# zrudnick/bramble

Hardware: AMD Instinct MI355X
Metric: projected alignments/sec vs GENCODE-scale annotation (higher is better)
Workload: dtype u32; 1 GPU; device-resident (inputs already in HBM, packed rows left in HBM): 10M paired-end 2x100 short reads (name-collated, unstranded) vs GENCODE-shaped synthetic annotation (250836 transcripts, 1684128 transcript-exon rows, 25 refs); BASELINE.json configs[1]; group_lanes=8, seed=0xb4a3b1e

## Files before the change

### bramble_amd/csrc/kernels.h

```cpp
#pragma once
#include <hip/hip_runtime.h>
#include <stdint.h>

#include "device_types.h"
#include "ksw_types.h"

namespace br {

enum {
  TOT_MATCHES = 0,
  TOT_ARENA = 1,
  TOT_SIMPLE = 2,
  TOT_ROWS = 3,
  TOT_RAW = 4,
  TOT_RESCUE_PROB = 5,
  TOT_RESCUE_SEQ = 6,
  TOT_WIDE_CIGAR = 7,
  TOT_SMALL_CNT = 8,
  TOT_PARSE_CIGAR = 12,
  TOT_PARSE_NAMES = 13,
  TOT_PARSE_GROUPS = 14,
  TOT_PARSE_SEQ = 15,
  TOT_BAM_LONG = 16,
  TOT_BAM_BYTES = 17,
// ... 6 lines not shown

struct ProjectArgs {
  DevIndex ix;
  DevCfg cfg;
  int64_t n_aln;
  const int32_t *ref_id;
  const uint32_t *cigar_off;
  const uint32_t *cigar;
  const uint2 *seg;
  const AlnMeta *meta;
  const uint4 *head;
  const uint4 *head2;
  const uint32_t *fast_flag;
  const uint32_t *fast_pre;
  uint32_t *n_matches;
  uint4 *ranges;
  uint64_t *mask;
  uint32_t *big_list;
  uint32_t *n_big;
  uint32_t *walk_list;
  uint32_t *n_walk;
  uint32_t *m_aln;
  const uint32_t *match_off;
  const uint64_t *cig_base;
  uint32_t *m_tid, *m_aux;
  uint2 *m_p;
  uint2 *m_x;
  uint4 *m_b;
  uint64_t *m_cigoff;
  uint32_t *cig_arena;
  const uint64_t *tot;
  uint64_t lim_m, lim_c;
  uint64_t cover;
};
__device__ __forceinline__ bool tot_over(const uint64_t *tot, uint64_t lim_m, uint64_t lim_c) { return tot && (tot[TOT_MATCHES] > lim_m || tot[TOT_ARENA] > lim_c); }

struct CountArgs {
  const uint32_t *slab_off, *bin_off, *s_start, *s_pmax;
  const uint4 *t_bin, *s_row, *tx_ex;
  uint32_t n_refs, bin_shift;
  uint32_t max_clip, max_junc_ins, max_junc_gap, max_error_exon;
  int32_t ignore_small_exons, long_reads;
  uint32_t n_aln;
  const uint4 *head, *head2;
  const uint32_t *cigar_off;
  const uint2 *seg;
  uint32_t *n_matches;
  uint64_t *mask;
  uint4 *ranges;
  uint32_t *walk_list, *n_walk;
  uint32_t *big_list, *n_big;
  uint32_t *light_flag;
};

struct FaArgs {
  const int32_t *seq_src;
  const uint32_t *seq_off;
  const uint8_t *seqs;
  uint32_t *n_prob;
  uint32_t *seq_bytes;
  const uint32_t *prob_off;
  const uint64_t *seqarena_off;
  KswProb *probs;
  FaSrc *srcs;
  KswRes *results;
  uint8_t *seq_arena;
  uint32_t *clip_ops;
  uint32_t *ideal_cap;
  uint64_t *want_l, *want_r;
};

struct KswArgs {
  int64_t n_prob;
  const KswProb *probs;
  KswRes *results;
  const uint8_t *seq_arena;
  uint32_t *clip_ops;
  uint8_t *scratch;
  size_t scratch_per_wave, pmat_bytes, raw_words;
  int64_t n_waves;
  uint32_t tmax;
  uint64_t *stats;
  uint32_t *raw_out, *raw_n; int32_t *max_out; uint32_t raw_cap;
  const uint32_t *list; const uint32_t *n_list;
};

struct KswFastArgs {
  int64_t p0, n;
  const KswProb *probs;
  KswRes *results;
  const uint8_t *seq_arena;
  uint32_t *clip_ops, *raw_ops;
  KswDesc *desc[KSW_N_BINS];
  uint32_t *counters;
  uint32_t *leftover;
  KswDp *dp;
  uint8_t *tape; uint64_t tape_cap;
  uint32_t n_bin[KSW_N_BINS], n_groups[KSW_N_BINS];
  uint64_t *stats;
  uint32_t *raw_out, *raw_n; int32_t *max_out; uint32_t raw_cap;
};

struct ScanArgs {
  int64_t n;
  const uint32_t *src32;
  const uint32_t *cigar_off;
// ... 213 lines not shown
void launch_split_emit(hipStream_t st, const SplitArgs &S);
void launch_split_totals(hipStream_t st, const SplitArgs &S);
void launch_last_group(hipStream_t st, const uint8_t *data, const uint64_t *rec_off, int64_t n, unsigned long long *out);
void launch_unmapped_before(hipStream_t st, const SplitArgs &S, uint64_t limit, unsigned long long *out);
void launch_first_record(hipStream_t st, const SplitArgs &S, uint64_t limit, unsigned long long *out);
void launch_piece_cut(hipStream_t st, const SplitArgs &S, const uint64_t *rec_off, int64_t n, uint64_t bound, uint64_t used, int guess, unsigned long long *cut);

struct ParseArgs {
  int64_t n, n_groups;
  const uint8_t *blob;
  const uint64_t *rec_off;
  const uint32_t *rec_len;
  const int32_t *ref_map;
  int32_t n_ref_map;
  int32_t *ref_id, *ref_start, *l_qseq;
  uint16_t *flags;
  uint32_t *ncig, *name_len, *isnew;
  uint32_t *maxima;
  const uint32_t *group_pre;
  uint32_t *group_off;
  const uint32_t *cigar_off, *name_off;
  uint32_t *cigar;
  uint8_t *names;
  int32_t *mate_idx;
  uint32_t *n_big_groups, *big_groups;
  int32_t *seq_src;
  uint32_t *seq_len;
  const uint32_t *seq_off;
  uint8_t *seqs;
  const int32_t *mate_ref_id, *mate_start;
};
struct SoaArgs {
  int64_t n;
  const uint64_t *cigar_off64, *name_off64, *seq_off64;
  uint32_t *cigar_off, *name_off, *seq_off;
  const uint8_t *names;
  const uint32_t *cigar;
  uint32_t *isnew;
  uint32_t *maxima;
};
void launch_soa_fields(hipStream_t st, const SoaArgs &S);
void launch_rec_fields(hipStream_t st, const ParseArgs &P);
void launch_group_off(hipStream_t st, const ParseArgs &P);
void launch_rec_copy(hipStream_t st, const ParseArgs &P);
void launch_mates(hipStream_t st, const ParseArgs &P);
void launch_seq_src(hipStream_t st, const ParseArgs &P);
void launch_seq_ascii(hipStream_t st, const ParseArgs &P);
void launch_bam_size(hipStream_t st, const BamArgs &B);
void launch_bam_encode(hipStream_t st, const BamArgs &B, int lanes);

struct SegExtra {
  const uint32_t *group_off; uint32_t *aln_group; int64_t n_groups;
  uint64_t *zero_a; int n_zero_a; uint64_t *zero_b; int n_zero_b;
};
void launch_segment(hipStream_t st, int64_t n_aln, const int32_t *ref_id, const int32_t *ref_start,
                    const uint16_t *flags, const int8_t *xs, const int8_t *ts, const uint32_t *cigar_off,
                    const uint32_t *cigar, const DevCfg &cfg, uint32_t n_refs, uint2 *seg, AlnMeta *meta,
                    uint4 *head, uint4 *head2, uint32_t *fast_flag, const SegExtra *extra = nullptr);
void launch_project(hipStream_t st, const ProjectArgs &A, bool emit, int group_lanes, int n_blocks);
void launch_count(hipStream_t st, const CountArgs &C, int group_lanes, int n_blocks, int part);
void launch_project_fa(hipStream_t st, const ProjectArgs &A, const FaArgs &F, int mode, int n_blocks);
void launch_fa_fill(hipStream_t st, const ProjectArgs &A, const FaArgs &F, int64_t n_prob);
void launch_ksw(hipStream_t st, const KswArgs &K, int n_blocks);
void launch_ksw_bin(hipStream_t st, const KswFastArgs &A);
void launch_ksw_dp(hipStream_t st, const KswFastArgs &A, int bin);
void launch_ksw_trace(hipStream_t st, const KswFastArgs &A, int bin);
uint32_t ksw_dp_resident_groups(int bin, int n_cu);
size_t ksw_prob_bytes();
size_t ksw_res_bytes();
void launch_expand(hipStream_t st, const ProjectArgs &A);
void launch_emit_dense(hipStream_t st, const ProjectArgs &A, int64_t n_matches, int64_t n_simple, int part);
void launch_emit_dense_fa(hipStream_t st, const ProjectArgs &A, const FaArgs &F, int64_t n_matches);
int64_t scan_tiles_for(int64_t n);
void launch_scan(hipStream_t st, const ScanArgs &S, int mode, void *out, bool out64, uint64_t *total_out);
void launch_group_ids(hipStream_t st, int64_t n_groups, const uint32_t *group_off, uint32_t *aln_group);
bool launch_scan3(hipStream_t st, ScanArgs S, uint32_t *match_off, uint64_t *cig_base, uint32_t *fast_pre,
                  uint64_t *total_out3, const ProjectArgs *expand = nullptr);
void launch_pair(hipStream_t st, const PairArgs &P, bool emit);
void launch_primary(hipStream_t st, const PairArgs &P, const uint32_t *name_off, const uint8_t *names, bool has_scores);
void launch_rows(hipStream_t st, const PairArgs &P, bool aux);
void launch_rows_detail(hipStream_t st, const PairArgs &P);
void launch_pool_sizes(hipStream_t st, const PoolArgs &Q);
void launch_pool_copy(hipStream_t st, const PoolArgs &Q, bool long_cigars);
void launch_wide_fields(hipStream_t st, const WideArgs &W);
void launch_wide_cigars(hipStream_t st, const WideArgs &W, int64_t n_words);

}
```

### bramble_amd/csrc/pipeline.cpp

```cpp
#include <algorithm>
#include <cstring>
#include <vector>

#include "ctx.h"

int ensure_side_stream(br_ctx *c) {
  if (c->side_stream) return BR_OK;
  HIPCHK(hipStreamCreateWithPriority(&c->side_stream, hipStreamNonBlocking, 0));
  for (auto &p : c->side_ev) for (auto &e : p) HIPCHK(hipEventCreateWithFlags(&e, hipEventDisableTiming));
  return BR_OK;
}

int run_ksw(br_ctx *c, hipStream_t st, const KswRun &R) {
  if (R.n_prob <= 0) return BR_OK;
  const uint64_t n_all = (uint64_t)R.n_prob;
  const uint64_t qmax = std::max<uint64_t>(R.qmax, 1), tmax = std::max<uint64_t>(R.tmax, 1);
  KswArgs K{};
  K.n_prob = R.n_prob; K.probs = R.probs; K.results = R.results; K.seq_arena = R.seq_arena; K.clip_ops = R.clip_ops;
  K.stats = R.stats;
  K.raw_out = R.raw_out; K.raw_n = R.raw_n; K.max_out = R.max_out; K.raw_cap = R.raw_cap;
  auto general = [&](uint64_t n_work, uint64_t q_hi, uint64_t t_hi, const uint32_t *list, const uint32_t *n_list) -> int {
    q_hi = std::max<uint64_t>(q_hi, 1); t_hi = std::max<uint64_t>(t_hi, 1);
    K.tmax = (uint32_t)t_hi;
    K.pmat_bytes = (size_t)(((q_hi + t_hi) * t_hi + 15) & ~15ull);
// ... 362 lines not shown
  HIPCHK(hipMemcpyAsync(rb->small, d_tot, sizeof(rb->small), hipMemcpyDeviceToHost, st));
  HIPCHK(hipStreamSynchronize(st));
  for (int k = 0; k < 4; k++) { rb->scan[k] = rb->small[k]; rb->counters[k] = rb->small[TOT_SMALL_CNT + k]; }
  const uint64_t n_matches = rb->scan[TOT_MATCHES], n_cig_arena = rb->scan[TOT_ARENA], n_simple = rb->scan[TOT_SIMPLE], n_rows = rb->scan[TOT_ROWS];
  if (n_matches > cap_m || n_cig_arena > cap_c || n_rows > P.lim_r) return BR_RETRY_ORDINARY;
  if (big && (!dc.filter_by_similarity ? (n_simple > cover_s || n_matches - n_simple > cover_g) : n_matches > cover_m)) return BR_RETRY_ORDINARY;
  c->hist_simf = dc.filter_by_similarity != 0;
  c->hist_n = n; c->hist[0] = n_matches; c->hist[1] = n_cig_arena; c->hist[2] = n_simple; c->hist[3] = n_rows;
  if (!keep_events) RC(pf.collect());
  if (rb->counters[3]) return BR_ERR_UNSUPPORTED;
  finish_call(c, dc, b, out, n_matches, n_rows, n_cig_arena, aux_cols, &P);
  return BR_OK;
}

static int run_device_direct(br_ctx *c, const DevCfg &dc, const br_device_batch *b, hipStream_t st, br_device_rows *out, Prof &pf,
                             bool keep_events) {
  const br_index *ix = c->ix;
  const int64_t n = b->n_aln, ng = b->n_groups;
  const int64_t tiles = std::max<int64_t>(scan_tiles_for(std::max<int64_t>(n, ng) + 1), 1);
  RC(ensure_count_tables(c, b));
  RC(c->n_matches.ensure((size_t)n * 4 + 16));
  RC(c->tile_sums.ensure((size_t)tiles * 8 * 5));
  RC(c->counters_d.ensure((GD_COUNTER_WORDS + 4) * 8));
  uint64_t *const dz = c->counters_d.as<uint64_t>();
  uint32_t *const dz_nbig = (uint32_t *)(dz + GD_COUNTER_WORDS + 2);
  RC(c->walk_list.ensure((size_t)n * 4));
  RC(c->aln_group.ensure((size_t)n * 4)); RC(c->n_rows.ensure((size_t)n * 4 + 16)); RC(c->pbit.ensure((size_t)n + 16));
  RC(c->d_fm.ensure((size_t)n * sizeof(uint2) + (size_t)(n / 62 + 2) * 4));
  RC(c->d_nkept.ensure((size_t)n * 4)); RC(c->d_desc.ensure((size_t)n * sizeof(uint4)));
  RC(c->d_hi0.ensure((size_t)n * 4)); RC(c->d_clspos.ensure((size_t)n * 4)); RC(c->d_rnd.ensure((size_t)std::max<int64_t>(ng, 1) * 8));
  if (c->d_side_cap == 0) c->d_side_cap = std::max<uint64_t>((uint64_t)n / 4, 1u << 20);
  RC(c->d_side.ensure((size_t)c->d_side_cap * sizeof(uint2)));
  if (c->rows_busy_set && c->row_off.cap < (size_t)(n + 1) * 8) HIPCHK(hipEventSynchronize(c->rows_busy));
  RC(c->row_off.ensure((size_t)(n + 1) * 8));
  RC(ensure_side_stream(c));
  if (!c->side2_stream) HIPCHK(hipStreamCreateWithPriority(&c->side2_stream, hipStreamNonBlocking, 0));
  hipStream_t ax = c->side_stream, ax2 = c->side2_stream;
  uint64_t *d_tot = c->totals.as<uint64_t>();
  ReadBack *rb = c->rb;

  ProjectArgs A = count_args(c, dc, b);
  A.n_big = dz_nbig; A.walk_list = c->walk_list.as<uint32_t>(); A.n_walk = dz_nbig + 1;
  const bool have_names = b->names && b->name_off;
  DirectArgs D{};
  D.n_aln = n; D.n_groups = ng; D.group_off = b->group_off; D.aln_group = c->aln_group.as<uint32_t>(); D.mate_idx = b->mate_idx;
  D.n_matches = c->n_matches.as<uint32_t>(); D.mask = c->mask.as<uint64_t>(); D.ranges = c->ranges.as<uint4>();
  D.fast_flag = c->fast_flag.as<uint32_t>(); D.s_tid = ix->dev.s_tid; D.big_list = A.big_list; D.n_big = A.n_big;
  D.fm = c->d_fm.as<uint2>(); D.pm_list = (uint32_t *)(c->d_fm.as<uint2>() + n); D.pm_n = dz_nbig + 2; D.n_kept = c->d_nkept.as<uint32_t>(); D.n_rows = c->n_rows.as<uint32_t>(); D.pflag = c->pbit.as<uint8_t>();
  D.side = c->d_side.as<uint2>(); D.side_cap = c->d_side_cap; D.side_used = (unsigned long long *)(dz + GD_COUNTER_WORDS);
  D.cls_pos = c->d_clspos.as<uint32_t>(); D.cig_base = c->cig_base.as<uint64_t>(); D.row_off = c->row_off.as<uint64_t>();
  D.name_off = have_names ? b->name_off : nullptr; D.names = have_names ? b->names : nullptr; D.rnd0 = c->d_rnd.as<uint64_t>();
  D.gd = c->d_desc.as<uint2>(); D.dpos = c->d_desc.as<uint2>() + n; D.hi0 = c->d_hi0.as<uint32_t>(); D.counters = c->counters_d.as<uint64_t>(); D.tot = d_tot;

  SideWork seeds(c, st, ax2), pair_big(c, st, ax), group_desc(c, st, ax), big_emit(c, st, ax);
  HIPCHK(hipMemsetAsync(dz, 0, (GD_COUNTER_WORDS + 4) * 8, st));
  RC(pair_big.fork());
  RC(segment_stage(c, st, dc, b, pf));
  RC(pf.begin(BR_K_GROUP_IDS));
  launch_group_ids(st, ng, b->group_off, c->aln_group.as<uint32_t>());
  RC(pf.end());
  RC(count_pass(c, st, A, pf, true, true));
  if (c->rows_busy_set) { HIPCHK(hipStreamWaitEvent(st, c->rows_busy, 0)); }
  const int big_blocks = c->n_cu * 4;
  uint64_t kept = 0, arena = 0, n_simple = 0, n_rows = 0, n_raw = 0;
  bool expanded_ahead = false;
  if (have_names) {
    RC(seeds.fork());
    RC(pf.begin(BR_K_NAME_SEED, ax2));
    launch_name_seed(ax2, D);
    RC(pf.end());
    RC(seeds.done());
  }
  for (int attempt = 0;; attempt++) {
    if (attempt) {
      HIPCHK(hipMemsetAsync(dz, 0, (GD_COUNTER_WORDS + 2) * 8, st));
      HIPCHK(hipMemsetAsync(D.pm_n, 0, 4, st));
    }
    RC(pair_big.fork());
    RC(pf.begin(BR_K_PAIR_BIG, ax));
    launch_big_collect(ax, A, D, big_blocks);
    launch_pair_big(ax, D, big_blocks);
    RC(pf.end());
    RC(pair_big.done());
    RC(pf.begin(BR_K_PAIR_MASK));
    launch_pair_mask(st, D, c->n_cu * 2);
    RC(pf.end());
    RC(pair_big.join());
    RC(group_desc.fork());
    if (have_names) RC(seeds.join_on(ax));
    RC(pf.begin(BR_K_GROUP_DESC, ax));
    launch_group_desc(ax, D);
    RC(pf.end());
    RC(group_desc.done());
    RC(pf.begin(BR_K_SCAN));
    launch_scan5(st, D, c->tile_sums.as<uint64_t>(), d_tot);
    RC(pf.end());
    expanded_ahead = false;
    if (c->m_aln.cap >= 4) {
      D.m_aln = c->m_aln.as<uint32_t>(); D.m_aln_cap = c->m_aln.cap / 4;
      RC(pf.begin(BR_K_EXPAND_ROWS));
      launch_expand_rows(st, D);
      RC(pf.end());
      expanded_ahead = true;
    }
    HIPCHK(hipMemcpyAsync(rb->scan, d_tot, sizeof(rb->scan), hipMemcpyDeviceToHost, st));
    HIPCHK(hipMemcpyAsync(rb->side, dz + GD_COUNTER_WORDS, sizeof(rb->side), hipMemcpyDeviceToHost, st));
    HIPCHK(hipStreamSynchronize(st));
    c->d_side_attempts = attempt + 1;
    if (rb->side[1]) {
      if (attempt >= 3) return BR_ERR_CAPACITY;
      RC(group_desc.wait_host());
      c->d_side_cap = rb->side[0] + rb->side[0] / 4 + 4096;
      RC(c->d_side.ensure((size_t)c->d_side_cap * sizeof(uint2)));
      D.side = c->d_side.as<uint2>(); D.side_cap = c->d_side_cap;
      continue;
    }
    kept = rb->scan[TOT_MATCHES]; arena = rb->scan[TOT_ARENA]; n_simple = rb->scan[TOT_SIMPLE]; n_rows = rb->scan[TOT_ROWS]; n_raw = rb->scan[TOT_RAW];
    break;
  }
  if (n_raw >= 0xffffffffull || kept >= 0xffffffffull) return BR_ERR_CAPACITY;
  if (kept != n_rows) return BR_ERR_HIP;

  const size_t nr = (size_t)std::max<uint64_t>(n_rows, 1);
  if (c->rows_busy_set && (c->pk_a.cap < nr * sizeof(uint4) || c->pk_c.cap < nr * sizeof(uint2))) HIPCHK(hipEventSynchronize(c->rows_busy));
  RC(c->pk_a.ensure(nr * sizeof(uint4))); RC(c->pk_c.ensure(nr * sizeof(uint2)));
  if (expanded_ahead && kept > D.m_aln_cap) expanded_ahead = false;
  RC(c->m_aln.ensure(nr * 4)); RC(c->cig_arena.ensure((size_t)std::max<uint64_t>(arena, 1) * 4));
  const bool with_x = c->want_x;
  if (with_x) {
    if (c->rows_busy_set && c->pk_x.cap < nr * sizeof(uint4)) HIPCHK(hipEventSynchronize(c->rows_busy));
    RC(c->pk_x.ensure(nr * sizeof(uint4)));
  }
  A.cig_arena = c->cig_arena.as<uint32_t>();
  D.m_aln = c->m_aln.as<uint32_t>(); D.r_a = c->pk_a.as<uint4>(); D.r_c = c->pk_c.as<uint2>(); D.r_x = with_x ? c->pk_x.as<uint4>() : nullptr;
  D.m_aln_cap = 0;
  if (kept) {
    if (!expanded_ahead) {
      RC(pf.begin(BR_K_EXPAND_ROWS));
      launch_expand_rows(st, D);
      RC(pf.end());
    }
    RC(group_desc.join());
    RC(big_emit.fork());
    RC(pf.begin(BR_K_BIG_EMIT, ax));
    launch_big_emit(ax, A, D, big_blocks);
    RC(pf.end());
    RC(big_emit.done());
    RC(pf.begin(BR_K_EMIT_ROWS_SIMPLE));
    launch_emit_rows(st, A, D, (int64_t)kept, (int64_t)n_simple, 1);
    RC(pf.end());
    RC(pf.begin(BR_K_EMIT_ROWS));
    launch_emit_rows(st, A, D, (int64_t)kept, (int64_t)n_simple, 2);
    RC(pf.end());
    RC(big_emit.join());
  } else {
    RC(group_desc.join());
  }
  HIPCHK(hipMemcpyAsync(rb->direct_cnt, c->counters_d.p, sizeof(rb->direct_cnt), hipMemcpyDeviceToHost, st));
  HIPCHK(hipStreamSynchronize(st));
  if (!keep_events) RC(pf.collect());
  for (int k = 0; k < 4; k++) rb->counters[k] = rb->direct_cnt[k];
  for (int k = 0; k < GD_SLOTS; k++) { rb->counters[1] += rb->direct_cnt[GD_SLOT0 + k * GD_SLOT_STRIDE]; rb->counters[2] += rb->direct_cnt[GD_SLOT0 + k * GD_SLOT_STRIDE + 1]; }
  if (rb->counters[3]) return BR_ERR_UNSUPPORTED;
  c->hist_n = 0;
  finish_call(c, dc, b, out, n_raw, n_rows, arena, false);
  out->a = (const br_row_a *)c->pk_a.p; out->cigar = (const uint64_t *)c->pk_c.p; out->x = with_x ? (const br_row_x *)c->pk_x.p : nullptr;
  out->similarity_score = nullptr; out->clip_score = nullptr;
  c->detail_valid = with_x;
  c->last_direct = true; c->dA = A; c->dD = D; c->d_kept = (int64_t)kept; c->d_simple = (int64_t)n_simple;
  return BR_OK;
}

static int run_match_table(br_ctx *c, const DevCfg &dc, const br_device_batch *b, hipStream_t st, br_device_rows *out, Prof &pf,
                           bool keep_events) {
// ... 254 lines not shown
}

extern "C" int br_ctx_collect_counters(br_ctx *c, const br_device_batch *b, void *stream) {
  if (!c || !b) return BR_ERR_INVALID_ARG;
  hipStream_t st = (hipStream_t)stream;
  HIPCHK(hipSetDevice(c->ix->device));
  if (c->last_direct) {
    const DevCfg dc = c->dA.cfg;
    Prof pf{c, st};
    c->events_used = 0;
    br_device_rows tmp;
    memset(&tmp, 0, sizeof(tmp));
    RC(run_match_table(c, dc, b, st, &tmp, pf, false));
  }
  DevBuf stats; RC(stats.ensure(8 * 8));
  HIPCHK(hipMemsetAsync(stats.p, 0, 8 * 8, st));
  StatsArgs T{};
  T.ix = c->ix->dev; T.n_aln = b->n_aln; T.ref_id = b->ref_id; T.cigar_off = b->cigar_off;
  T.seg = c->seg.as<uint2>(); T.head = c->head.as<uint4>(); T.head2 = c->head2.as<uint4>(); T.out = stats.as<uint64_t>();
  int64_t nm = (int64_t)c->counters[6];
  launch_stats(st, T, nm ? c->m_p.as<uint2>() : nullptr, c->match_off.as<uint32_t>(), c->n_matches.as<uint32_t>());
  uint64_t h[8];
  HIPCHK(hipMemcpyAsync(h, stats.p, 8 * 8, hipMemcpyDeviceToHost, st));
  HIPCHK(hipStreamSynchronize(st));
  uint64_t n = (uint64_t)b->n_aln;
  c->counters[3] = h[3]; c->counters[4] = h[4]; c->counters[5] = h[5]; c->counters[7] = h[7];
  c->counters[0] = 24ull * n + 4ull * h[3];
  c->counters[1] = h[1];
  c->counters[2] = 4ull * n + 24ull * (uint64_t)nm + 4ull * h[7];
  return BR_OK;
}

extern "C" int br_ctx_direct_diag(br_ctx *c, uint64_t out[8], uint8_t *pflags) {
  if (!c || !out || !c->last_direct) return BR_ERR_INVALID_ARG;
  HIPCHK(hipSetDevice(c->ix->device));
  const DirectArgs &D = c->dD;
  uint64_t used = 0;
  uint32_t nb[3] = {0, 0, 0};
  HIPCHK(hipDeviceSynchronize());
  HIPCHK(hipMemcpy(&used, D.side_used, 8, hipMemcpyDeviceToHost));
  HIPCHK(hipMemcpy(nb, D.n_big, 12, hipMemcpyDeviceToHost));
  if (pflags && D.n_aln > 0) HIPCHK(hipMemcpy(pflags, D.pflag, (size_t)D.n_aln, hipMemcpyDeviceToHost));
  memset(out, 0, 8 * sizeof(uint64_t));
  out[0] = nb[0]; out[1] = (uint64_t)c->d_side_attempts; out[2] = used; out[3] = D.side_cap; out[4] = nb[2];
  if (D.n_aln > 0) {
    const size_t n = (size_t)D.n_aln;
    std::vector<uint32_t> ff(n), nk(n);
    std::vector<uint4> hd(n);
    std::vector<uint8_t> pf(n);
    HIPCHK(hipMemcpy(ff.data(), D.fast_flag, n * 4, hipMemcpyDeviceToHost));
    HIPCHK(hipMemcpy(nk.data(), D.n_kept, n * 4, hipMemcpyDeviceToHost));
    HIPCHK(hipMemcpy(hd.data(), c->head.p, n * sizeof(uint4), hipMemcpyDeviceToHost));
    HIPCHK(hipMemcpy(pf.data(), D.pflag, n, hipMemcpyDeviceToHost));
    uint64_t light = 0;
    for (size_t a = 0; a < n; a++)
      if ((ff[a] >> 31) && hd[a].z == 2 && !(pf[a] & PF_BIG)) light += nk[a];
    out[5] = light;
  }
  return BR_OK;
}

extern "C" int br_project_batch_device(br_ctx *c, const br_config *cfg, const br_device_batch *b, void *stream,
                                       br_device_rows *out) {
  if (!c || !cfg || !b || !out) return BR_ERR_INVALID_ARG;
  return run_device(c, cfg, b, (hipStream_t)stream, out);
}

extern "C" int br_device_rows_expand(br_ctx *c, void *stream, br_device_wide_rows *out) {
  if (!c || !out) return BR_ERR_INVALID_ARG;
  return expand_rows(c, (hipStream_t)stream, out);
}
```

### bramble_amd/csrc/project_kernels.hip

```cpp
#include <hip/hip_runtime.h>
#include <stdint.h>

#include <algorithm>

#include "device_types.h"
#include "kernels.h"
#include "primary_pick.h"

namespace br {

#define CIG_OP(c) ((c) & 0xfu)
#define CIG_LEN(c) ((c) >> 4)
#define CIG_GEN(l, o) (((l) << 4) | (o))

__global__ void __launch_bounds__(256) k_segment(int64_t n_aln, const int32_t *__restrict__ ref_id,
                                                 const int32_t *__restrict__ ref_start,
                                                 const uint16_t *__restrict__ flags,
                                                 const int8_t *__restrict__ xs, const int8_t *__restrict__ ts,
                                                 const uint32_t *__restrict__ cigar_off,
                                                 const uint32_t *__restrict__ cigar, DevCfg cfg,
                                                 uint32_t n_refs, uint2 *__restrict__ seg,
                                                 AlnMeta *__restrict__ meta, uint4 *__restrict__ head,
                                                 uint4 *__restrict__ head2, uint32_t *__restrict__ fast_flag, SegExtra X) {
  int64_t a = (int64_t)blockIdx.x * blockDim.x + threadIdx.x;
// ... 32 lines not shown
        l += (int)len; exstart = pos0 + l; intron = true;
        break;
      case OP_S: case OP_H: ins = false; break;
      default: break;
    }
  }
  if (!intron) {
    ex_start = (uint32_t)(exstart + 1); ex_end = (uint32_t)(pos0 + l);
    const uint2 v = make_uint2(ex_start, ex_end + 1);
    if (n == 0) e0 = v; else if (n == 1) e1 = v; else if (n == 2) e2 = v;
    else { if (n == 3) { out[0] = e0; out[1] = e1; out[2] = e2; } out[n] = v; }
    n++;
  }
  if (ex_end == 0) n = 0;
  int32_t rid = ref_id[a];
  if (rid < 0 || (uint32_t)rid >= n_refs) n = 0;

  uint32_t smode = 3;
  uint16_t f = flags[a];
  if (!cfg.long_reads) {
    char c = (char)xs[a];
    if (c == 0) {
      char m = (char)ts[a];
      if (m == '+' || m == '-') c = (f & 0x10) ? ((m == '+') ? '-' : '+') : m;
    }
    char strand = (c == '+' || c == '-') ? c : '.';
    if (strand == '.' && (cfg.fr || cfg.rf)) {
      bool is_rev = f & 0x10;
      bool cond = (cfg.rf && is_rev) || (cfg.fr && !is_rev);
      if (f & 0x1) {
        int order = (f & 0x40) ? 1 : ((f & 0x80) ? 2 : 0);
        strand = (order == 1) ? (cond ? '-' : '+') : (cond ? '+' : '-');
      } else {
        strand = cond ? '-' : '+';
      }
    }
    smode = (strand == '+') ? 1u : (strand == '-') ? 2u : 3u;
  }
  uint32_t lclip = 0, rclip = 0;
  if (cfg.long_reads) {
    if (n_cigar == 0) { n = 0; }
    else {
      uint32_t w0 = cg[0];
      if (CIG_OP(w0) == OP_H) { if (n_cigar > 1 && CIG_OP(cg[1]) == OP_S) lclip = CIG_LEN(cg[1]); }
      else if (CIG_OP(w0) == OP_S) lclip = CIG_LEN(w0);
      uint32_t wl = cg[n_cigar - 1];
      if (CIG_OP(wl) == OP_H) { if (n_cigar >= 2 && CIG_OP(cg[n_cigar - 2]) == OP_S) rclip = CIG_LEN(cg[n_cigar - 2]); }
      else if (CIG_OP(wl) == OP_S) rclip = CIG_LEN(wl);
    }
  }
  if (cfg.long_reads) { AlnMeta m; m.n_seg = n; m.smode = smode; m.n_left_clip = lclip; m.n_right_clip = rclip; meta[a] = m; }
  uint2 q0 = n ? e0 : make_uint2(0, 0);
  head[a] = make_uint4(q0.x, q0.y, n, n ? (((uint32_t)rid << 2) | smode) : 0u);
  if (n > 1) {
    const bool mnm = n == 2 && n_cigar == 3 && pre4 && CIG_OP(w4[0]) == OP_M && CIG_OP(w4[2]) == OP_M && !cfg.filter_by_similarity &&
                     !cfg.long_reads && !cfg.ignore_small_exons;
    const uint2 q2 = n > 2 ? e2 : make_uint2(mnm ? 1u : 0u, 0);
    head2[a] = make_uint4(e1.x, e1.y, q2.x, q2.y);
  }
  uint32_t fast = (n == 1 && n_cigar == 1 && CIG_OP(cg[0]) == OP_M && !cfg.filter_by_similarity && !cfg.long_reads) ? 1u : 0u;
  fast_flag[a] = (fast << 31) | ((n_cigar + 2u * (4u * n + 2u)) & 0x7fffffffu);
}

struct Hit { uint32_t pos, left_ins, right_ins, left_gap, right_gap; };

__device__ __forceinline__ bool classify(bool minus, int status, uint32_t qs, uint32_t qe, uint32_t s,
                                         uint32_t e, uint32_t pos_start, const DevCfg &c, Hit &h) {
  const bool junc_left = (status == ST_MIDDLE || status == ST_LAST);
  const bool junc_right = (status == ST_FIRST || status == ST_MIDDLE);
  const uint32_t lg = qs > s ? qs - s : 0u, li = s > qs ? s - qs : 0u;
  const uint32_t rg = e > qe ? e - qe : 0u, ri = qe > e ? qe - e : 0u;
  const uint32_t lim_li = junc_left ? c.max_junc_ins : c.max_clip;
  const uint32_t lim_ri = (junc_right || minus) ? c.max_junc_ins : c.max_clip;
  const uint32_t lim_lg = junc_left ? c.max_junc_gap : 0xffffffffu;
  const uint32_t lim_rg = junc_right ? c.max_junc_gap : 0xffffffffu;
  h.pos = pos_start + (minus ? rg : lg); h.left_ins = li; h.right_ins = ri; h.left_gap = lg; h.right_gap = rg;
  return (li <= lim_li) & (ri <= lim_ri) & (lg <= lim_lg) & (rg <= lim_rg);
}

struct IdealSink {
  uint32_t *buf; uint32_t n; uint32_t cur; bool has;
  __device__ __forceinline__ void init(uint32_t *b) { buf = b; n = 0; cur = 0; has = false; }
  __device__ __forceinline__ void add(uint32_t len, uint32_t op) {
    const bool same = has && CIG_OP(cur) == op;
    const bool flush = has && !same;
    if (flush && buf) buf[n] = cur;
    n += flush ? 1u : 0u;
    cur = same ? cur + (len << 4) : CIG_GEN(len, op);
    has = true;
  }
  __device__ __forceinline__ uint32_t finish() { if (has) { if (buf) buf[n] = cur; n++; has = false; } return n; }
};

struct Acc {
  double cov, ops;
  int32_t ref_consumed, junc_hits, clip_score;
  uint32_t prev_op;
  uint32_t last_pos;
  __device__ __forceinline__ void init() { cov = 0; ops = 0; ref_consumed = 0; junc_hits = 0; clip_score = 0; prev_op = OP_M; last_pos = 0; }
};

__device__ __forceinline__ void build_match(Acc &m, IdealSink &sk, const Hit &h, int status, uint32_t qs,
                                            uint32_t qe, uint32_t gs, uint32_t ge, bool first_match,
                                            bool last_match, bool has_lc, bool has_rc) {
  if (h.left_ins > 0) {
    if (status == ST_FIRST || status == ST_ONLY) {
      if (!has_lc) { sk.add(h.left_ins, OP_S); m.ops += h.left_ins; m.prev_op = OP_S; }
    } else {
      sk.add(h.left_ins, OP_I); m.ops += h.left_ins;
      if (m.prev_op == OP_D) m.cov += h.left_ins;
      else if (m.prev_op == OP_I) m.ops += (m.ops * 0.2);
      m.prev_op = OP_I;
    }
// ... 632 lines not shown
              uint32_t k = aux_n + (uint32_t)__popcll(m & ((1ull << gl) - 1ull));
              A.m_aux[moff + k] = pay.x;
            }
            aux_n += (uint32_t)__popcll(m);
          } else if (alive) {
            for (uint32_t k = 0; k < aux_n; k++) rank += (A.m_aux[moff + k] < pay.x) ? 1u : 0u;
            do_emit = true;
          }
        }
        if constexpr (EMIT) {
          if (!do_emit) continue;
          uint32_t *slot = A.cig_arena + cbase + (uint64_t)rank * cap;
          uint32_t *lds = &sh_cig[(EMIT ? threadIdx.x : 0) * LDS_SLOT];
          bool ideal_lds = ideal_cap <= LDS_IDEAL;
          uint32_t *ideal = ideal_lds ? lds : slot + rd.n_real + ideal_cap;
          sk.init(ideal);
          walk_pass2(ix, cfg, rd, E, s == 1, sb[s], se[s], i0, q0, make_uint4(gs, gend, pay.z, 0), make_uint2(nxt, nxe), h0, p1, acc, sk, no_clip(), no_clip());
          uint32_t n_ideal = sk.finish();
          similarity(cfg, acc, score);
          bool out_lds = ideal_lds && (rd.n_real + n_ideal <= LDS_SLOT - LDS_IDEAL);
          uint32_t *outp = out_lds ? lds + LDS_IDEAL : slot;
          RealCig rc; rc.fetch(rd.real, rd.n_real);
          uint32_t n_out = merge_cigars(rc, rd.n_real, ideal, n_ideal, outp);
          uint64_t cig_ref = cbase + (uint64_t)rank * cap;
          if (n_out <= 2) cig_ref = (uint64_t)(n_out > 0 ? outp[0] : 0u) | ((uint64_t)(n_out > 1 ? outp[1] : 0u) << 32);
          else if (out_lds) for (uint32_t k = 0; k < n_out; k++) slot[k] = outp[k];
          uint32_t mi = moff + rank;
          A.m_tid[mi] = pay.x;
          A.m_p[mi] = make_uint2((s == 0) ? p1.fwpos : p1.rcpos, n_out | ((uint32_t)s << 31));
          A.m_x[mi] = make_uint2((uint32_t)acc.junc_hits, (uint32_t)acc.ref_consumed);
          if (SIMF) {
            unsigned long long sb64 = (unsigned long long)__double_as_longlong(score);
            A.m_b[mi] = make_uint4((uint32_t)acc.clip_score, 0u, (uint32_t)sb64, (uint32_t)(sb64 >> 32));
          }
          A.m_cigoff[mi] = cig_ref;
        }
      }
      if (EMIT && !have_mask && sweep == 0) __threadfence_block();
    }
    if (MODE == 1 && ((__ballot(defer) >> gbase) & gmask) != 0) {
      if (gl == 0) {
        uint32_t k = atomicAdd(&sh_wn, 1u);
        if (k < WALK_LDS) sh_wl[MODE == 1 ? k : 0] = (uint32_t)a;
        else { uint32_t k2 = atomicAdd(A.n_walk, 1u); A.walk_list[k2] = (uint32_t)a; }
      }
      continue;
    }
    bool light = false;
    if constexpr (MODE == 1 && CNT && PRE == 1)
      light = n_seg == 2 && hd2.z != 0 && n_items <= 64 && ((__ballot(inexact != 0u) >> gbase) & gmask) == 0;
    if (!EMIT && gl == 0) {
      A.n_matches[a] = total; A.mask[a] = mask_all;
      if constexpr (MODE == 1 && CNT && PRE == 1) { if (light && A.light_flag) A.light_flag[a] = (1u << 31) | (3u + 2u * (4u * 2u + 2u)); }
      if (n_items > 64 && total) {
        const uint32_t k = atomicAdd(&sh_bn, 1u);
        if (k < BIG_LDS) sh_bl[EMIT ? 0 : k] = (uint32_t)a;
        else { const uint32_t k2 = atomicAdd(A.n_big, 1u); A.big_list[k2] = (uint32_t)a; }
      }
    }
  }
  if (!EMIT) {
    __syncthreads();
    const uint32_t n_loc = sh_bn < BIG_LDS ? sh_bn : BIG_LDS;
    if (threadIdx.x == 0) sh_bbase = n_loc ? atomicAdd(A.n_big, n_loc) : 0u;
    __syncthreads();
    for (uint32_t i = threadIdx.x; i < n_loc; i += blockDim.x) A.big_list[sh_bbase + i] = sh_bl[EMIT ? 0 : i];
  }
  if (MODE == 1) {
    __syncthreads();
    const uint32_t n_loc = sh_wn < WALK_LDS ? sh_wn : WALK_LDS;
    if (threadIdx.x == 0) sh_wbase = n_loc ? atomicAdd(A.n_walk, n_loc) : 0u;
    __syncthreads();
    for (uint32_t i = threadIdx.x; i < n_loc; i += blockDim.x) A.walk_list[sh_wbase + i] = sh_wl[MODE == 1 ? i : 0];
  }
}

__device__ __forceinline__ void expand_chunk(const ProjectArgs &A, int64_t a, uint32_t (*sh_pre)[64], uint32_t (*sh_v)[64]) {
  const int lane = threadIdx.x & 63, wv = threadIdx.x >> 6;
  uint32_t nm = 0, pos = 0, v = 0;
  bool fast = false;
  if (a < A.n_aln) nm = A.n_matches[a];
  if (nm) {
    const uint32_t fp = A.fast_pre[a];
    fast = A.fast_flag[a] >> 31;
    pos = fast ? fp : A.fast_pre[A.n_aln] + (A.match_off[a] - fp);
    const uint4 rg = A.ranges[a];
    const uint32_t n_items = (rg.y - rg.x) + (rg.w - rg.z);
    v = n_items <= 64 ? (uint32_t)a : 0xffffffffu;
  }
  sh_v[wv][lane] = v;
#pragma unroll
  for (int c = 0; c < 2; c++) {
    const uint32_t mine = (nm && fast == (c == 0)) ? nm : 0u;
    const uint64_t have = __ballot(mine != 0u);
    if (!have) continue;
    uint32_t inc = mine;
#pragma unroll
    for (int d = 1; d < 64; d <<= 1) { const uint32_t up = __shfl_up(inc, d); if (lane >= d) inc += up; }
    const uint32_t total = __shfl(inc, 63), first = __shfl(pos, (int)__builtin_ctzll(have));
    __builtin_amdgcn_wave_barrier();
    sh_pre[wv][lane] = inc - mine;
    __builtin_amdgcn_fence(__ATOMIC_RELEASE, "workgroup");
    __builtin_amdgcn_wave_barrier();
    __builtin_amdgcn_fence(__ATOMIC_ACQUIRE, "workgroup");
    for (uint32_t e = lane; e < total; e += 64) {
      int l = 0;
// ... 893 lines not shown

static inline int grid_for(int64_t n, int per_block) { return (int)((n + per_block - 1) / per_block); }

void launch_segment(hipStream_t st, int64_t n_aln, const int32_t *ref_id, const int32_t *ref_start,
                    const uint16_t *flags, const int8_t *xs, const int8_t *ts, const uint32_t *cigar_off,
                    const uint32_t *cigar, const DevCfg &cfg, uint32_t n_refs, uint2 *seg, AlnMeta *meta,
                    uint4 *head, uint4 *head2, uint32_t *fast_flag, const SegExtra *extra) {
  if (n_aln <= 0) return;
  SegExtra X{};
  if (extra) X = *extra;
  hipLaunchKernelGGL(k_segment, dim3(grid_for(n_aln, 256)), dim3(256), 0, st, n_aln, ref_id, ref_start, flags,
                     xs, ts, cigar_off, cigar, cfg, n_refs, seg, meta, head, head2, fast_flag, X);
}

template <int G>
static void launch_project_g(hipStream_t st, const ProjectArgs &A, bool emit, int n_blocks) {
  bool simf = A.cfg.filter_by_similarity != 0;
  if (emit) {
    if (simf) hipLaunchKernelGGL((k_project<G, true, true>), dim3(n_blocks), dim3(256), 0, st, A);
    else hipLaunchKernelGGL((k_project<G, true, false>), dim3(n_blocks), dim3(256), 0, st, A);
  } else {
    if (simf) hipLaunchKernelGGL((k_project<G, false, true>), dim3(n_blocks), dim3(256), 0, st, A);
    else hipLaunchKernelGGL((k_project<G, false, false>), dim3(n_blocks), dim3(256), 0, st, A);
  }
}

static int project_blocks(int64_t n_aln, int group_lanes, int n_blocks) {
  const int per_block = 256 / group_lanes;
  const int64_t need = (n_aln + per_block - 1) / per_block;
  if (need < n_blocks) n_blocks = (int)need;
  return n_blocks < 1 ? 1 : n_blocks;
}

void launch_project(hipStream_t st, const ProjectArgs &A, bool emit, int group_lanes, int n_blocks) {
  if (!emit && A.ix.n_rows == 0) {
    (void)hipMemsetAsync(A.n_matches, 0, (size_t)A.n_aln * 4, st);
    (void)hipMemsetAsync(A.mask, 0, (size_t)A.n_aln * 8, st);
    (void)hipMemsetAsync(A.ranges, 0, (size_t)A.n_aln * sizeof(uint4), st);
    return;
  }
  if (A.n_aln <= 0) return;
  n_blocks = project_blocks(A.n_aln, group_lanes, n_blocks);
  switch (group_lanes) {
    case 8: launch_project_g<8>(st, A, emit, n_blocks); break;
    case 16: launch_project_g<16>(st, A, emit, n_blocks); break;
    case 32: launch_project_g<32>(st, A, emit, n_blocks); break;
    default: launch_project_g<64>(st, A, emit, n_blocks); break;
  }
}

template <int G>
static void launch_count_g(hipStream_t st, const CountArgs &C, int n_blocks, int part) {
  const bool pre = !C.long_reads && !C.ignore_small_exons;
  const dim3 g(n_blocks), b(256);
  if (part == 1) {
    if (pre) hipLaunchKernelGGL((k_project<G, false, false, 1, 1, CountArgs>), g, b, 0, st, C);
    else hipLaunchKernelGGL((k_project<G, false, false, 1, 0, CountArgs>), g, b, 0, st, C);
  } else {
    if (pre) hipLaunchKernelGGL((k_project<G, false, false, 2, 1, CountArgs>), g, b, 0, st, C);
    else hipLaunchKernelGGL((k_project<G, false, false, 2, 0, CountArgs>), g, b, 0, st, C);
  }
}

void launch_count(hipStream_t st, const CountArgs &C, int group_lanes, int n_blocks, int part) {
  if (C.n_aln == 0) return;
  n_blocks = project_blocks(C.n_aln, group_lanes, n_blocks);
  switch (group_lanes) {
    case 8: launch_count_g<8>(st, C, n_blocks, part); break;
    case 16: launch_count_g<16>(st, C, n_blocks, part); break;
    case 32: launch_count_g<32>(st, C, n_blocks, part); break;
    default: launch_count_g<64>(st, C, n_blocks, part); break;
  }
}

void launch_expand(hipStream_t st, const ProjectArgs &A) {
  if (A.n_aln <= 0) return;
  hipLaunchKernelGGL(k_expand, dim3(grid_for(A.n_aln, 256)), dim3(256), 0, st, A);
}

void launch_emit_dense(hipStream_t st, const ProjectArgs &A0, int64_t n_matches, int64_t n_simple, int part) {
  if (A0.n_aln <= 0 || n_matches <= 0) return;
  ProjectArgs A = A0;
  if (A.tot) A.cover = (uint64_t)(part == 1 ? n_simple : part == 2 ? n_matches - n_simple : n_matches);
  const FaArgs F{};
  if (A.cfg.filter_by_similarity) { hipLaunchKernelGGL((k_emit_dense<true, 0>), dim3(grid_for(n_matches, 256)), dim3(256), 0, st, A, (int64_t)0, n_matches, F); return; }
  if (part == 0 || n_simple < 0) { hipLaunchKernelGGL((k_emit_dense<false, 0>), dim3(grid_for(n_matches, 256)), dim3(256), 0, st, A, (int64_t)0, n_matches, F); return; }
  if (part == 1) { if (n_simple > 0) hipLaunchKernelGGL((k_emit_dense<false, 1>), dim3(grid_for(n_simple, 256)), dim3(256), 0, st, A, (int64_t)0, n_simple, F); }
  else if (n_matches > n_simple) hipLaunchKernelGGL((k_emit_dense<false, 2>), dim3(grid_for(n_matches - n_simple, 256)), dim3(256), 0, st, A, n_simple, n_matches, F);
}

void launch_emit_dense_fa(hipStream_t st, const ProjectArgs &A, const FaArgs &F, int64_t n_matches) {
  if (A.n_aln <= 0 || n_matches <= 0) return;
  hipLaunchKernelGGL((k_emit_dense<true, 0, true>), dim3(grid_for(n_matches, 256)), dim3(256), 0, st, A, (int64_t)0, n_matches, F);
}

int64_t scan_tiles_for(int64_t n) { return (n + SCAN_TILE - 1) / SCAN_TILE; }

void launch_scan(hipStream_t st, const ScanArgs &S, int mode, void *out, bool out64, uint64_t *total_out) {
  int64_t tiles = scan_tiles_for(S.n);
  if (tiles < 1) tiles = 1;
  dim3 g((unsigned)tiles), b(256);
  if (tiles <= SCAN_SMALL_TILES) {
    const dim3 one(1);
    if (mode == 1) hipLaunchKernelGGL((k_scan_small<1, uint64_t>), one, b, 0, st, S, (uint64_t *)out, total_out);
    else if (mode == 3) hipLaunchKernelGGL((k_scan_small<3, uint64_t>), one, b, 0, st, S, (uint64_t *)out, total_out);
    else if (out64) hipLaunchKernelGGL((k_scan_small<2, uint64_t>), one, b, 0, st, S, (uint64_t *)out, total_out);
    else hipLaunchKernelGGL((k_scan_small<2, uint32_t>), one, b, 0, st, S, (uint32_t *)out, total_out);
    return;
// ... 94 lines not shown
```

### bramble_amd/lib.py

```python
import ctypes as C
import os

import numpy as np

_HERE = os.path.dirname(os.path.abspath(__file__))
LIB_PATH = os.path.join(_HERE, "libbramble_amd.so")
_P = C.POINTER

K_SEGMENT, K_COUNT, K_EMIT, K_PAIR_COUNT, K_PAIR_EMIT, K_GATHER, K_SCAN, K_EMIT_AUX, K_KSW, K_BAM, K_PARSE, K_CODEC, K_EMIT_SIMPLE, K_PRIMARY, K_CIGAR_POOL, K_COUNT_WALK, K_EXPAND, K_GROUP_IDS, K_P1, K_P1_WALK, K_EMIT_WL, K_NAME_SEED, K_PAIR_MASK, K_PAIR_BIG, K_GROUP_DESC, K_EXPAND_ROWS, K_EMIT_ROWS_SIMPLE, K_EMIT_ROWS, K_BIG_EMIT, K_SAM_FORMAT, K_NUM = range(31)
KERNEL_NAMES = ["k_segment", "k_project<G,false,false,1>", "k_emit_dense<false,2>", "k_pair<false>", "k_pair<true>",
                "k_rows", "k_scan_*", "k_project<64,true>", "k_ksw", "k_bam_scan+k_bam_size+k_bam_encode",
                "k_rec_fields+k_group_off+k_rec_copy+k_mates+k_seq_*", "k_deflate_*+k_bgzf_compact",
                "k_emit_dense<false,1>", "k_primary", "(unused)", "k_project<G,false,false,2>", "k_expand", "k_group_ids",
                "(unused)", "(unused)", "(unused)", "k_name_seed", "k_pair_mask", "k_big<0>+k_pair_big", "k_group_desc",
                "k_expand_rows", "k_emit_rows<1>", "k_emit_rows<2>", "k_big<1>", "k_samfmt_*"]


class BrambleError(RuntimeError):
    pass


class BrExon(C.Structure):
    _fields_ = [("start", C.c_uint32), ("end", C.c_uint32)]

# ... 492 lines not shown
        return out

    def project_batch(self, cfg, batch):
        keep = []
        b = _batch_struct(batch, keep)
        r = BrRows()
        check(lib().br_project_batch(self.h, C.byref(cfg), C.byref(b), C.byref(r)), "br_project_batch")
        n = r.n_rows
        rows = {"n_rows": n}
        for name, dt in _ROW_FIELDS + [("is_primary", np.uint8)] + _ROW_TAIL:
            if name == "cigar_off":
                rows[name] = _view(r.cigar_off, n + 1, dt)
            elif name == "cigar":
                continue
            else:
                rows[name] = _view(getattr(r, name), n, dt)
        rows["cigar"] = _view(r.cigar, int(rows["cigar_off"][-1]) if n else 0, np.uint32)
        for name, _ in _COUNTERS:
            rows[name] = int(getattr(r, name))
        return rows

    @staticmethod
    def _device_batch_struct(dev_batch):
        db = BrDeviceBatch()
        db.n_aln = dev_batch["n_aln"]
        db.n_groups = dev_batch["n_groups"]
        for name in ("ref_id", "ref_start", "flags", "xs", "ts", "cigar_off", "cigar", "mate_idx", "group_off",
                     "l_qseq"):
            setattr(db, name, dev_batch[name].data_ptr())
        db.n_cigar_words = dev_batch["n_cigar_words"]
        db.max_n_cigar = dev_batch["max_n_cigar"]
        if dev_batch.get("seqs") is not None:
            db.seq_off = dev_batch["seq_off"].data_ptr()
            db.seqs = dev_batch["seqs"].data_ptr()
            db.seq_src = dev_batch["seq_src"].data_ptr()
            db.max_soft_clip = dev_batch["max_soft_clip"]
        if dev_batch.get("names") is not None:
            db.name_off = dev_batch["name_off"].data_ptr()
            db.names = dev_batch["names"].data_ptr()
        return db

    def collect_counters(self, dev_batch, stream=0):
        db = self._device_batch_struct(dev_batch)
        check(lib().br_ctx_collect_counters(self.h, C.byref(db), C.c_void_p(stream)), "br_ctx_collect_counters")
        out = (C.c_uint64 * 8)()
        check(lib().br_ctx_last_counters(self.h, out), "br_ctx_last_counters")
        keys = ("B_in", "B_idx", "B_out", "n_cigar", "read_exons", "overlap_hits", "matches", "out_cigar_words")
        return dict(zip(keys, [int(v) for v in out]))

    def direct_diag(self, n_aln=None):
        out = (C.c_uint64 * 8)()
        pf = np.zeros(n_aln, dtype=np.uint8) if n_aln is not None else None
        check(lib().br_ctx_direct_diag(self.h, out, pf.ctypes.data if pf is not None and n_aln else None), "br_ctx_direct_diag")
        d = dict(zip(("n_big", "side_attempts", "side_used", "side_cap", "pm_n", "light"), [int(v) for v in out[:6]]))
        if pf is not None:
            d["pflags"] = pf
        return d

    def project_bam_device(self, cfg, blob, rec_off, rec_len, ref_map, stream=0):
        recs = BrDeviceRecords()
        recs.blob = blob.data_ptr()
        recs.rec_off = rec_off.data_ptr()
        recs.n_aln = rec_len.numel()
        recs.rec_len = rec_len.data_ptr()
        rm = np.ascontiguousarray(ref_map, dtype=np.int32)
        rows, out = BrDeviceRows(), BrDeviceBam()
        check(lib().br_project_bam_device(self.h, C.byref(cfg), C.byref(recs), rm.ctypes.data, len(rm), C.c_void_p(stream),
                                          C.byref(rows), C.byref(out)), "br_project_bam_device")
        return rows, out

    def bgzf_deflate_device(self, src, stream=0):
        import torch
        from .device import _DevArray
        out, n = C.c_void_p(), C.c_uint64()
        check(lib().br_bgzf_deflate_device(self.h, C.c_void_p(src.data_ptr()), src.numel(), C.c_void_p(stream), C.byref(out),
                                           C.byref(n)), "br_bgzf_deflate_device")
        if n.value == 0:
            return torch.zeros(0, dtype=torch.uint8, device=src.device)
        return torch.as_tensor(_DevArray(out.value, n.value, "|u1"), device=src.device)

    def bgzf_inflate_device(self, src, blocks, stream=0):
        import torch
        from .device import _DevArray
        out, n = C.c_void_p(), C.c_uint64()
        blocks = np.ascontiguousarray(blocks, dtype=BGZF_BLOCK)
        L = lib()
        L.br_bgzf_inflate_device.argtypes = [C.c_void_p, C.c_void_p, C.c_uint64, C.c_void_p, C.c_int64, C.c_void_p, _P(C.c_void_p), _P(C.c_uint64)]
        check(L.br_bgzf_inflate_device(self.h, C.c_void_p(src.data_ptr()), src.numel(), C.c_void_p(blocks.ctypes.data), len(blocks),
                                       C.c_void_p(stream), C.byref(out), C.byref(n)), "br_bgzf_inflate_device")
        if n.value == 0:
            return torch.zeros(0, dtype=torch.uint8, device=src.device)
        return torch.as_tensor(_DevArray(out.value, n.value, "|u1"), device=src.device)

    def set_sam_refs(self, names):
        arr = (C.c_char_p * max(len(names), 1))(*[n.encode() if isinstance(n, str) else bytes(n) for n in names])
        L = lib()
        L.br_ctx_set_sam_refs.argtypes = [C.c_void_p, C.c_void_p, C.c_int32]
        check(L.br_ctx_set_sam_refs(self.h, arr, len(names)), "br_ctx_set_sam_refs")

    def sam_format_device(self, data, row_off=None, stream=0):
        import torch
        from .device import _DevArray
        if isinstance(data, BrDeviceBam):
            db, dev = data, torch.device("cuda", torch.cuda.current_device())
        else:
            db, dev = BrDeviceBam(), data.device
            db.data, db.n_bytes = data.data_ptr() if data.numel() else None, data.numel()
# ... 556 lines not shown
```

Before: 3.103 billion alignments/s.

## Route M-N-M spliced reads through lean count path and async totals readback

Segment stage now marks two-segment M-N-M alignments as fast (light) when the config is lean, and a new lean count-kernel variant (PRE=2) sets the light flag for such reads so they can take the cheap emit path. The totals/side readback moves to a side stream with a host wait on that stream only, letting the expand kernel keep running on the main stream during the host round-trip. Error paths now synchronize the main stream before returning. It also adds diagnostics (big_light, n_walk) and profiling scripts. Risks include mis-classifying spliced reads and stream-ordering hazards on the retry path.

Measured after the change: 3.071 billion alignments/s. 0.99x the previous value.

```diff
diff --git a/bramble_amd/csrc/kernels.h b/bramble_amd/csrc/kernels.h
--- a/bramble_amd/csrc/kernels.h
+++ b/bramble_amd/csrc/kernels.h
@@ -82,6 +82,9 @@
   uint32_t *big_list, *n_big;
   uint32_t *light_flag;
 };
+inline bool count_pass_lean(int32_t long_reads, int32_t ignore_small_exons, uint32_t max_junc_ins, uint32_t max_junc_gap) {
+  return !long_reads && !ignore_small_exons && max_junc_ins == 0 && max_junc_gap == 0;
+}
 
 struct FaArgs {
   const int32_t *seq_src;
@@ -401,6 +404,7 @@
 struct SegExtra {
   const uint32_t *group_off; uint32_t *aln_group; int64_t n_groups;
   uint64_t *zero_a; int n_zero_a; uint64_t *zero_b; int n_zero_b;
+  int mark_mnm;
 };
 void launch_segment(hipStream_t st, int64_t n_aln, const int32_t *ref_id, const int32_t *ref_start,
                     const uint16_t *flags, const int8_t *xs, const int8_t *ts, const uint32_t *cigar_off,
diff --git a/bramble_amd/csrc/pipeline.cpp b/bramble_amd/csrc/pipeline.cpp
--- a/bramble_amd/csrc/pipeline.cpp
+++ b/bramble_amd/csrc/pipeline.cpp
@@ -438,10 +438,12 @@
   D.name_off = have_names ? b->name_off : nullptr; D.names = have_names ? b->names : nullptr; D.rnd0 = c->d_rnd.as<uint64_t>();
   D.gd = c->d_desc.as<uint2>(); D.dpos = c->d_desc.as<uint2>() + n; D.hi0 = c->d_hi0.as<uint32_t>(); D.counters = c->counters_d.as<uint64_t>(); D.tot = d_tot;
 
-  SideWork seeds(c, st, ax2), pair_big(c, st, ax), group_desc(c, st, ax), big_emit(c, st, ax);
+  SideWork seeds(c, st, ax2), pair_big(c, st, ax), group_desc(c, st, ax), big_emit(c, st, ax), totals(c, st, ax2);
   HIPCHK(hipMemsetAsync(dz, 0, (GD_COUNTER_WORDS + 4) * 8, st));
   RC(pair_big.fork());
-  RC(segment_stage(c, st, dc, b, pf));
+  SegExtra X{};
+  X.mark_mnm = count_pass_lean(dc.long_reads, dc.ignore_small_exons, dc.max_junc_ins, dc.max_junc_gap) && A.ix.n_rows != 0;
+  RC(segment_stage(c, st, dc, b, pf, &X));
   RC(pf.begin(BR_K_GROUP_IDS));
   launch_group_ids(st, ng, b->group_off, c->aln_group.as<uint32_t>());
   RC(pf.end());
@@ -481,6 +483,7 @@
     RC(pf.begin(BR_K_SCAN));
     launch_scan5(st, D, c->tile_sums.as<uint64_t>(), d_tot);
     RC(pf.end());
+    RC(totals.fork());
     expanded_ahead = false;
     if (c->m_aln.cap >= 4) {
       D.m_aln = c->m_aln.as<uint32_t>(); D.m_aln_cap = c->m_aln.cap / 4;
@@ -489,12 +492,14 @@
       RC(pf.end());
       expanded_ahead = true;
     }
-    HIPCHK(hipMemcpyAsync(rb->scan, d_tot, sizeof(rb->scan), hipMemcpyDeviceToHost, st));
-    HIPCHK(hipMemcpyAsync(rb->side, dz + GD_COUNTER_WORDS, sizeof(rb->side), hipMemcpyDeviceToHost, st));
-    HIPCHK(hipStreamSynchronize(st));
+    HIPCHK(hipMemcpyAsync(rb->scan, d_tot, sizeof(rb->scan), hipMemcpyDeviceToHost, ax2));
+    HIPCHK(hipMemcpyAsync(rb->side, dz + GD_COUNTER_WORDS, sizeof(rb->side), hipMemcpyDeviceToHost, ax2));
+    RC(totals.done());
+    RC(totals.wait_host());
     c->d_side_attempts = attempt + 1;
     if (rb->side[1]) {
-      if (attempt >= 3) return BR_ERR_CAPACITY;
+      if (attempt >= 3) { HIPCHK(hipStreamSynchronize(st)); return BR_ERR_CAPACITY; }
+      HIPCHK(hipStreamSynchronize(st));
       RC(group_desc.wait_host());
       c->d_side_cap = rb->side[0] + rb->side[0] / 4 + 4096;
       RC(c->d_side.ensure((size_t)c->d_side_cap * sizeof(uint2)));
@@ -504,8 +509,8 @@
     kept = rb->scan[TOT_MATCHES]; arena = rb->scan[TOT_ARENA]; n_simple = rb->scan[TOT_SIMPLE]; n_rows = rb->scan[TOT_ROWS]; n_raw = rb->scan[TOT_RAW];
     break;
   }
-  if (n_raw >= 0xffffffffull || kept >= 0xffffffffull) return BR_ERR_CAPACITY;
-  if (kept != n_rows) return BR_ERR_HIP;
+  if (n_raw >= 0xffffffffull || kept >= 0xffffffffull) { HIPCHK(hipStreamSynchronize(st)); return BR_ERR_CAPACITY; }
+  if (kept != n_rows) { HIPCHK(hipStreamSynchronize(st)); return BR_ERR_HIP; }
 
   const size_t nr = (size_t)std::max<uint64_t>(n_rows, 1);
   if (c->rows_busy_set && (c->pk_a.cap < nr * sizeof(uint4) || c->pk_c.cap < nr * sizeof(uint2))) HIPCHK(hipEventSynchronize(c->rows_busy));
@@ -866,10 +871,12 @@
     HIPCHK(hipMemcpy(nk.data(), D.n_kept, n * 4, hipMemcpyDeviceToHost));
     HIPCHK(hipMemcpy(hd.data(), c->head.p, n * sizeof(uint4), hipMemcpyDeviceToHost));
     HIPCHK(hipMemcpy(pf.data(), D.pflag, n, hipMemcpyDeviceToHost));
-    uint64_t light = 0;
-    for (size_t a = 0; a < n; a++)
+    uint64_t light = 0, big_light = 0;
+    for (size_t a = 0; a < n; a++) {
       if ((ff[a] >> 31) && hd[a].z == 2 && !(pf[a] & PF_BIG)) light += nk[a];
-    out[5] = light;
+      if ((ff[a] >> 31) && hd[a].z == 2 && (pf[a] & PF_BIG)) big_light++;
+    }
+    out[5] = light; out[6] = big_light; out[7] = nb[1];
   }
   return BR_OK;
 }
diff --git a/bramble_amd/csrc/project_kernels.hip b/bramble_amd/csrc/project_kernels.hip
--- a/bramble_amd/csrc/project_kernels.hip
+++ b/bramble_amd/csrc/project_kernels.hip
@@ -108,13 +108,14 @@
   if (cfg.long_reads) { AlnMeta m; m.n_seg = n; m.smode = smode; m.n_left_clip = lclip; m.n_right_clip = rclip; meta[a] = m; }
   uint2 q0 = n ? e0 : make_uint2(0, 0);
   head[a] = make_uint4(q0.x, q0.y, n, n ? (((uint32_t)rid << 2) | smode) : 0u);
+  const bool mnm = n == 2 && n_cigar == 3 && pre4 && CIG_OP(w4[0]) == OP_M && CIG_OP(w4[2]) == OP_M && !cfg.filter_by_similarity &&
+                   !cfg.long_reads && !cfg.ignore_small_exons;
   if (n > 1) {
-    const bool mnm = n == 2 && n_cigar == 3 && pre4 && CIG_OP(w4[0]) == OP_M && CIG_OP(w4[2]) == OP_M && !cfg.filter_by_similarity &&
-                     !cfg.long_reads && !cfg.ignore_small_exons;
     const uint2 q2 = n > 2 ? e2 : make_uint2(mnm ? 1u : 0u, 0);
     head2[a] = make_uint4(e1.x, e1.y, q2.x, q2.y);
   }
   uint32_t fast = (n == 1 && n_cigar == 1 && CIG_OP(cg[0]) == OP_M && !cfg.filter_by_similarity && !cfg.long_reads) ? 1u : 0u;
+  if (X.mark_mnm && mnm) fast = 1u;
   fast_flag[a] = (fast << 31) | ((n_cigar + 2u * (4u * n + 2u)) & 0x7fffffffu);
 }
 
@@ -853,6 +854,9 @@
     if (!EMIT && gl == 0) {
       A.n_matches[a] = total; A.mask[a] = mask_all;
       if constexpr (MODE == 1 && CNT && PRE == 1) { if (light && A.light_flag) A.light_flag[a] = (1u << 31) | (3u + 2u * (4u * 2u + 2u)); }
+      if constexpr (MODE != 0 && CNT && PRE == 2) {
+        if ((MODE == 2 || n_items > 64) && n_seg == 2 && hd2.z != 0 && A.light_flag) A.light_flag[a] = 3u + 2u * (4u * 2u + 2u);
+      }
       if (n_items > 64 && total) {
         const uint32_t k = atomicAdd(&sh_bn, 1u);
         if (k < BIG_LDS) sh_bl[EMIT ? 0 : k] = (uint32_t)a;
@@ -1852,8 +1856,12 @@
 template <int G>
 static void launch_count_g(hipStream_t st, const CountArgs &C, int n_blocks, int part) {
   const bool pre = !C.long_reads && !C.ignore_small_exons;
+  const bool lean = count_pass_lean(C.long_reads, C.ignore_small_exons, C.max_junc_ins, C.max_junc_gap);
   const dim3 g(n_blocks), b(256);
-  if (part == 1) {
+  if (lean) {
+    if (part == 1) hipLaunchKernelGGL((k_project<G, false, false, 1, 2, CountArgs>), g, b, 0, st, C);
+    else hipLaunchKernelGGL((k_project<G, false, false, 2, 2, CountArgs>), g, b, 0, st, C);
+  } else if (part == 1) {
     if (pre) hipLaunchKernelGGL((k_project<G, false, false, 1, 1, CountArgs>), g, b, 0, st, C);
     else hipLaunchKernelGGL((k_project<G, false, false, 1, 0, CountArgs>), g, b, 0, st, C);
   } else {
diff --git a/bramble_amd/lib.py b/bramble_amd/lib.py
--- a/bramble_amd/lib.py
+++ b/bramble_amd/lib.py
@@ -568,7 +568,7 @@
         out = (C.c_uint64 * 8)()
         pf = np.zeros(n_aln, dtype=np.uint8) if n_aln is not None else None
         check(lib().br_ctx_direct_diag(self.h, out, pf.ctypes.data if pf is not None and n_aln else None), "br_ctx_direct_diag")
-        d = dict(zip(("n_big", "side_attempts", "side_used", "side_cap", "pm_n", "light"), [int(v) for v in out[:6]]))
+        d = dict(zip(("n_big", "side_attempts", "side_used", "side_cap", "pm_n", "light", "big_light", "n_walk"), [int(v) for v in out[:8]]))
         if pf is not None:
             d["pflags"] = pf
         return d
diff --git a/profiles/emit_gap.py b/profiles/emit_gap.py
--- /dev/null
+++ b/profiles/emit_gap.py
@@ -0,0 +1,19 @@
+#!/usr/bin/env python3
+import csv
+import sys
+if len(sys.argv) != 2:
+    sys.exit("usage: profiles/emit_gap.py KERNEL_TRACE_CSV")
+ends, gaps = None, []
+rows = sorted(csv.DictReader(open(sys.argv[1])), key=lambda r: int(r["Start_Timestamp"]))
+for r in rows:
+    name = r["Kernel_Name"]
+    if "k_expand_rows" in name:
+        ends = int(r["End_Timestamp"])
+    elif "k_emit_rows<1>" in name and ends is not None:
+        gaps.append((int(r["Start_Timestamp"]) - ends) / 1e3)
+        ends = None
+if not gaps:
+    sys.exit("no k_expand_rows -> k_emit_rows<1> pair in " + sys.argv[1])
+gaps.sort()
+n = len(gaps)
+print("k_expand_rows end -> k_emit_rows<1> start, us: n %d min %.1f median %.1f max %.1f" % (n, gaps[0], gaps[n // 2], gaps[-1]))
diff --git a/profiles/light_count.py b/profiles/light_count.py
--- /dev/null
+++ b/profiles/light_count.py
@@ -0,0 +1,14 @@
+#!/usr/bin/env python3
+import sys
+sys.path.insert(0, ".")
+from bramble_amd import lib, synth
+ann = synth.Annotation("G", n_genes=1500, n_refs=3)
+idx = lib.Index(ann.as_dict(), device=0)
+for mode in ("pe", "se"):
+    batch = ann.reads(20000, mode)
+    for lanes in (8, 64):
+        ctx = lib.Context(idx)
+        ctx.set_param("small_batch", 0); ctx.set_param("direct_rows", 1); ctx.set_param("group_lanes", lanes)
+        rows = ctx.project_batch(lib.make_config(), batch)
+        print("LIGHT", mode, lanes, ctx.direct_diag()["light"], rows["n_rows"], flush=True)
+        ctx.close()
```
